# discord/lilliput

Measured on NVIDIA H100. Metric: images_per_sec_1080p_jpeg_to_256x256_jpeg_q85, higher is better.
Workload: dtype u8

## Files before the change

lilliput_b200/csrc/abi_opencv.cu:

```cuda
#include <algorithm>
#include <cstring>
#include <memory>
#include <mutex>
#include <new>
#include <string>
#include <vector>

#include "common.cuh"
#include "kernels.cuh"
#include "lp_opencv.h"

namespace lp {

thread_local long g_launches = 0;

static std::once_flag g_dev_once;
static int g_dev_status = LP_ERR_CUDA;

int ensure_device() {
    std::call_once(g_dev_once, [] {
        int n = 0;
        cudaError_t e = cudaGetDeviceCount(&n);
        if (e != cudaSuccess || n == 0) {
            fprintf(stderr,
// ... 140 lines not shown
        sets.resize(kMultiscanMaxSets);
        int rc = jpeg_parse_scans(d->data, d->len, h, scans.data(), (int)scans.size(), &nscans, sets.data(),
                                  (int)sets.size(), &nsets);
        if (rc) return rc;
        const size_t visits = jpeg_multiscan_visits(h, scans.data(), nscans);
        if (visits > kMultiscanMaxVisits) {
            fprintf(stderr, "[lilliput_b200] multi-scan JPEG: %zu block visits over %d scans exceed the serial decoder's budget\n",
                    visits, nscans);
            return LP_ERR_UNSUPPORTED;
        }
    }
    cudaStream_t st = thread_stream();
    JpegDecodeItem it;
    memset(&it, 0, sizeof(it));
    it.scan_off = 0;
    it.scan_len = (uint32_t)h.scan_length;
    it.table_set = 0;
    it.width = h.width;
    it.height = h.height;
    it.ncomp = h.ncomp;
    it.mcus_x = h.mcus_x;
    it.mcus_y = h.mcus_y;
    it.restart_interval = h.restart_interval;
    uint32_t total_blocks = 0;
    for (int c = 0; c < h.ncomp; c++) {
        it.h[c] = h.comp[c].h;
        it.v[c] = h.comp[c].v;
        it.dw[c] = (h.width * h.comp[c].h + h.maxh - 1) / h.maxh;
        it.dh[c] = (h.height * h.comp[c].v + h.maxv - 1) / h.maxv;
        total_blocks += (uint32_t)h.mcus_x * h.mcus_y * h.comp[c].h * h.comp[c].v;
        memcpy(it.qt[c], h.qt[h.comp[c].tq], sizeof(it.qt[c]));
        it.td[c] = h.comp[c].td;
        it.ta[c] = h.comp[c].ta;
    }
    uint32_t tiles = 0;
    const uint32_t blocks = jpeg_item_set_window(&it, 0, 0, h.width, h.height, false, &tiles);
    if (h.multiscan) {
        it.restart_interval = 0;
        it.table_set = 0;
        it.nscans = (uint32_t)nscans;
    }
    it.frame_channels = h.ncomp == 1 ? 1 : 3;
    JpegHuffSet hs;
    jpeg_build_huff_set(h, &hs);

    uint8_t* scratch = nullptr;
    const size_t upload_len = h.multiscan ? d->len : h.scan_length;
    const size_t scan_bytes = round_up(upload_len + 16, (size_t)256);
    const size_t sets_b = round_up(sizeof(JpegHuffSet) * (size_t)(h.multiscan ? nsets : 1), (size_t)256);
    const size_t scans_b = round_up(sizeof(JpegScanDesc) * (size_t)nscans + 16, (size_t)256);
    const size_t coef_bytes = round_up((size_t)blocks * 64 * sizeof(int16_t), (size_t)256);
    const bool parallel = h.restart_interval == 0 && !h.multiscan;
    const size_t clean_b = parallel ? round_up(huff_clean_bytes(h.scan_length), (size_t)256) : 0;
    const size_t states_b = parallel ? round_up(2 * huff_nsub(h.scan_length) * 8, (size_t)256) : 0;
    const size_t nslots_b = parallel ? round_up(2 * huff_nsub(h.scan_length) * 4, (size_t)256) : 0;
    const size_t dcdiff_b = parallel ? round_up((size_t)total_blocks * 2, (size_t)256) : 0;
    const size_t total = 1024 + sets_b + scan_bytes + coef_bytes + clean_b + states_b + nslots_b +
                         dcdiff_b + scans_b;
    LP_CUDA_OK(cudaMallocAsync(&scratch, total, st));
    JpegDecodeItem* d_item = reinterpret_cast<JpegDecodeItem*>(scratch);
    JpegHuffSet* d_hs = reinterpret_cast<JpegHuffSet*>(scratch + 1024);
    uint8_t* d_scan = scratch + 1024 + sets_b;
    int16_t* d_coef = reinterpret_cast<int16_t*>(d_scan + scan_bytes);
    uint8_t* d_clean = reinterpret_cast<uint8_t*>(d_coef) + coef_bytes;
    uint8_t* d_states = d_clean + clean_b;
    uint8_t* d_nslots = d_states + states_b;
    uint8_t* d_dcdiff = d_nslots + nslots_b;
    JpegScanDesc* d_scans = reinterpret_cast<JpegScanDesc*>(d_dcdiff + dcdiff_b);
    LP_CUDA_OK(cudaMemcpyAsync(d_item, &it, sizeof(it), cudaMemcpyHostToDevice, st));
    if (h.multiscan) {
        LP_CUDA_OK(cudaMemcpyAsync(d_hs, sets.data(), sizeof(JpegHuffSet) * nsets, cudaMemcpyHostToDevice, st));
        LP_CUDA_OK(cudaMemcpyAsync(d_scans, scans.data(), sizeof(JpegScanDesc) * nscans, cudaMemcpyHostToDevice, st));
        LP_CUDA_OK(cudaMemcpyAsync(d_scan, d->data, d->len, cudaMemcpyHostToDevice, st));
    } else {
        LP_CUDA_OK(cudaMemcpyAsync(d_hs, &hs, sizeof(hs), cudaMemcpyHostToDevice, st));
        LP_CUDA_OK(cudaMemcpyAsync(d_scan, d->data + h.scan_offset, h.scan_length, cudaMemcpyHostToDevice, st));
    }
    JpegDecodeBatch b;
    b.items = d_item;
    b.tables = d_hs;
    b.scan = d_scan;
    b.coef = d_coef;
    b.frames = m->dptr();
    b.n = 1;
    b.coef_elems_total = (size_t)blocks * 64;
    b.max_tiles_per_image = (int)tiles;
    b.use_parallel_huffman = parallel;
    b.clean = d_clean;
    b.states = d_states;
    b.nslots = reinterpret_cast<uint32_t*>(d_nslots);
    b.dcdiff = reinterpret_cast<int16_t*>(d_dcdiff);
    if (h.multiscan) {
        b.n_multiscan = 1;
        b.scans = d_scans;
    }
    int rc = jpeg_decode_launch(b, st, nullptr);
    JpegDecodeItem back;
    if (!rc) {
        LP_CUDA_OK(cudaMemcpyAsync(&back, d_item, sizeof(back), cudaMemcpyDeviceToHost, st));
        rc = sync_stream();
    }
    cudaFreeAsync(scratch, st);
    if (rc) return rc;
    return back.status == 0 ? LP_OK : LP_ERR_DECODING_FAILED;
}

static int decode_png_into(const Decoder* d, Mat* m) {
    const PngHeader& h = d->png;
// ... 666 lines not shown
```

lilliput_b200/csrc/batch.cu:

```cuda
#include <algorithm>
#include <cstring>
#include <map>
#include <string>
#include <thread>
#include <unordered_map>
#include <utility>
#include <vector>

#include "common.cuh"
#include "kernels.cuh"
#include "lilliput_host.hpp"

using namespace lp;

static constexpr int kScansPerImage = 16, kSetsPerImage = 10;

namespace lp {
size_t batch_multiscan_pool_bytes(size_t n) {
    return ((kSetsPerImage * n + kMultiscanMaxSets) * sizeof(JpegHuffSet) +
            (kScansPerImage * n + kMultiscanMaxScans) * sizeof(JpegScanDesc));
}
}

struct lp_batch {
// ... 124 lines not shown
        return nullptr;
    }
    const int slots = jpeg_huff_parallel_slots();
    b->chunk = cfg->chunk > 0 ? cfg->chunk : (slots > 0 ? 3 * slots : 512);
    b->first_chunk = slots > 0 ? std::min(slots, b->chunk) : b->chunk / 2;
    b->pipe_chunk = (cfg->chunk > 0 || slots <= 0) ? b->chunk : std::min(b->chunk, 2 * slots);
    b->chunk = std::min(b->chunk, cfg->max_images);
    b->pipe_chunk = std::max(1, std::min(b->pipe_chunk, b->chunk));
    b->max_chunks = ceil_div(cfg->max_images, b->pipe_chunk) + 3;
    const size_t mcus = (size_t)ceil_div(b->W, 8) * ceil_div(b->H, 8);
    b->max_blocks_alloc = mcus * 3 + 4 * ((size_t)ceil_div(b->W, 8) + ceil_div(b->H, 8)) + 16;
    const size_t max_blocks = b->max_blocks_alloc;
    b->frame_bytes = (size_t)b->W * b->H * 3;
    b->resized_bytes = (size_t)b->out_w * b->out_h * 3;
    const size_t N = cfg->max_images;
    auto fail = [&]() -> lp_batch* { batch_free(b); return nullptr; };
#define BALLOC(ptr, bytes)                                                                      \
    if (dev_arena) {                                                                            \
        const size_t need_ = round_up((size_t)(bytes), (size_t)256);                            \
        if (dev_used + need_ > dev_bytes) return fail();                                        \
        (ptr) = reinterpret_cast<decltype(ptr)>(dev_arena + dev_used);                          \
        dev_used += need_;                                                                      \
    } else if (cudaMalloc(&(ptr), (bytes)) != cudaSuccess) {                                    \
        fprintf(stderr, "[lilliput_b200] lp_batch_create: cudaMalloc(%zu) failed\n", (size_t)(bytes)); \
        return fail();                                                                          \
    }
#define HALLOC(ptr, bytes)                                                                      \
    if (host_arena) {                                                                           \
        const size_t need_ = round_up((size_t)(bytes), (size_t)256);                            \
        if (host_used + need_ > host_bytes) return fail();                                      \
        (ptr) = reinterpret_cast<decltype(ptr)>(host_arena + host_used);                        \
        host_used += need_;                                                                     \
    } else if (cudaMallocHost(&(ptr), (bytes)) != cudaSuccess) {                                \
        return fail();                                                                          \
    }
    if (cudaStreamCreateWithFlags(&b->st, cudaStreamNonBlocking) != cudaSuccess) return fail();
    if (cudaStreamCreateWithFlags(&b->st_h2d, cudaStreamNonBlocking) != cudaSuccess) return fail();
    if (cudaStreamCreateWithFlags(&b->st_d2h, cudaStreamNonBlocking) != cudaSuccess) return fail();
    BALLOC(b->d_scan, cfg->max_in_bytes + 16 * N + 4096);
    BALLOC(b->d_items, N * sizeof(JpegDecodeItem));
    b->max_tables = (int)N;
    if (b->multiscan) {
        b->max_tables += (int)(kSetsPerImage * N) + kMultiscanMaxSets;
        b->max_scans = kScansPerImage * N + kMultiscanMaxScans;
        BALLOC(b->d_scans, b->max_scans * sizeof(JpegScanDesc));
        BALLOC(b->d_masks, (size_t)b->chunk * max_blocks * sizeof(uint64_t));
    }
    BALLOC(b->d_tables, (size_t)b->max_tables * sizeof(JpegHuffSet));
    BALLOC(b->d_coef, (size_t)b->chunk * max_blocks * 64 * sizeof(int16_t));
    BALLOC(b->d_frames, (size_t)b->chunk * b->frame_bytes + 256);
    BALLOC(b->d_resized, N * b->resized_bytes + 256);
    BALLOC(b->d_enc_scratch, jpeg_encode_scratch_bytes(b->out_w, b->out_h, 3, b->chunk, cfg->out_cap, b->progressive));
    BALLOC(b->d_clean, cfg->max_in_bytes + 64 * N + 4096);
    b->state_cap = (cfg->max_in_bytes / 128 + 2 * N + 16) * 2;
    BALLOC(b->d_states, b->state_cap * 8);
    BALLOC(b->d_nslots, b->state_cap * 4);
    BALLOC(b->d_dcdiff, (size_t)b->chunk * max_blocks * sizeof(int16_t));
    BALLOC(b->d_out, N * cfg->out_cap);
    BALLOC(b->d_out_len, N * sizeof(uint32_t));
#undef BALLOC
    HALLOC(b->h_out, N * cfg->out_cap);
    HALLOC(b->h_out_len, N * sizeof(uint32_t));
    HALLOC(b->h_items_back, N * sizeof(JpegDecodeItem));
    HALLOC(b->h_off, (N + (size_t)b->max_chunks + 8) * sizeof(unsigned long long));
#undef HALLOC
    b->ev.resize((size_t)b->max_chunks * 6);
    b->ev_h2d.resize(b->max_chunks);
    b->ev_d2h.resize(b->max_chunks);
    for (auto& e : b->ev)
        if (cudaEventCreate(&e) != cudaSuccess) return fail();
    for (auto& e : b->ev_h2d)
        if (cudaEventCreateWithFlags(&e, cudaEventDisableTiming) != cudaSuccess) return fail();
    for (auto& e : b->ev_d2h)
        if (cudaEventCreateWithFlags(&e, cudaEventDisableTiming) != cudaSuccess) return fail();
    b->items.resize(N);
    b->parse_status.resize(N);
    b->file_dev_off.resize(N);
    return b;
}

extern "C" void lp_batch_destroy(lp_batch* b) {
    if (!b) return;
    DeviceGuard dev_guard(b->cfg.device);
    cudaDeviceSynchronize();
    batch_free(b);
}

static int table_set_lookup(lp_batch* b, const JpegHeader& h);
static int table_set_for(lp_batch* b, const JpegHeader& h) {
    if (b->last_table_idx >= 0 && !memcmp(h.huff_present, b->last_present, sizeof(h.huff_present)) &&
        !memcmp(h.huff_bits, b->last_bits, sizeof(h.huff_bits)) && !memcmp(h.huff_vals, b->last_vals, sizeof(h.huff_vals)))
        return b->last_table_idx;
    const int found = table_set_lookup(b, h);
    if (found >= 0) {
        memcpy(b->last_present, h.huff_present, sizeof(h.huff_present));
        memcpy(b->last_bits, h.huff_bits, sizeof(h.huff_bits));
        memcpy(b->last_vals, h.huff_vals, sizeof(h.huff_vals));
        b->last_table_idx = found;
    }
    return found;
}

static int table_set_lookup(lp_batch* b, const JpegHeader& h) {
    std::string key;
    for (int tc = 0; tc < 2; tc++)
        for (int th = 0; th < 4; th++) {
            key.push_back((char)h.huff_present[tc][th]);
// ... 112 lines not shown
    lay.ordinal = ordinal;
    for (int k = i0; k < i0 + cnt; k++) {
        if (b->parse_status[k]) continue;
        const JpegDecodeItem& it = b->items[k];
        lay.blocks = std::max(lay.blocks, blocks_of[k - i0]);
        lay.tiles = std::max(lay.tiles, tiles_of[k - i0]);
        lay.total_blocks = std::max(lay.total_blocks, total_of[k - i0]);
        if (!b->layout_known) {
            b->win_w = it.win_w;
            b->win_h = it.win_h;
            b->win_x0 = it.win_x0;
            b->frame_bytes = (size_t)it.win_stride * it.win_h;
            b->layout_known = true;
        }
    }
    b->blocks = std::max(b->blocks, lay.blocks);
    b->total_blocks = std::max(b->total_blocks, lay.total_blocks);
    b->chunk_layout[i0] = lay;
    for (int k = i0; k < i0 + cnt; k++) {
        if (b->parse_status[k]) continue;
        JpegDecodeItem& it = b->items[k];
        const int slot = k - i0;
        if (!ms_scans[slot].empty()) {
            const std::vector<JpegScanDesc>& sc = ms_scans[slot];
            const std::vector<JpegHeader>& sets = ms_sets[slot];
            std::vector<int> global(sets.size(), -1);
            bool fits = b->scans.size() + sc.size() <= b->max_scans;
            for (size_t q = 0; q < sets.size() && fits; q++) fits = (global[q] = table_set_for(b, sets[q])) >= 0;
            if (!fits) {
                b->parse_status[k] = LP_ERR_UNSUPPORTED;
                it.status = -1;
                continue;
            }
            it.table_set = (uint32_t)b->scans.size();
            it.nscans = (uint32_t)sc.size();
            for (JpegScanDesc d : sc) {
                d.table_set = global[d.table_set];
                b->scans.push_back(d);
            }
            it.scan_off = b->file_dev_off[k];
            it.coef_off = (uint64_t)slot * lay.blocks * 64;
            it.frame_off = (uint64_t)slot * b->frame_bytes;
            it.dcdiff_off = (uint64_t)slot * lay.total_blocks;
            b->chunk_layout[i0].n_multiscan++;
            continue;
        }
        const int ts = table_set_for(b, hdr[k - i0]);
        if (ts < 0) {
            b->parse_status[k] = LP_ERR_UNSUPPORTED;
            it.status = -1;
            continue;
        }
        it.table_set = (uint32_t)ts;
        size_t state_need = 2 * huff_nsub(it.scan_len);
        if (it.restart_interval) {
            const uint32_t mcus = (uint32_t)it.mcus_x * it.mcus_y;
            const uint32_t nint = (mcus + (uint32_t)it.restart_interval - 1) / (uint32_t)it.restart_interval;
            it.clean_len = nint;
            state_need = std::max(state_need, (size_t)nint + 2);
            if (b->state_off + state_need > b->state_cap) {
                b->parse_status[k] = LP_ERR_UNSUPPORTED;
                it.status = -1;
                continue;
            }
            for (uint32_t q = 0; q < nint; q++) b->chunk_layout[i0].rst_work.push_back(make_uint2((unsigned)slot, q));
        }
        it.scan_off = b->file_dev_off[k] + hdr[k - i0].scan_offset;
        it.coef_off = (uint64_t)slot * lay.blocks * 64;
        it.frame_off = (uint64_t)slot * b->frame_bytes;
        it.dcdiff_off = (uint64_t)slot * lay.total_blocks;
        it.clean_off = b->clean_off;
        it.state_off = b->state_off;
        b->clean_off += huff_clean_bytes(it.scan_len);
        b->state_off += state_need;
    }
    return LP_OK;
}

static int batch_upload_files(lp_batch* b, const uint8_t* const* in, const size_t* in_len, int i0, int cnt,
                              cudaStream_t st) {
    int i = i0;
    while (i < i0 + cnt) {
        int j = i;
        size_t run = in_len[i];
        while (j + 1 < i0 + cnt && in[j + 1] == in[j] + in_len[j]) { j++; run += in_len[j]; }
        LP_CUDA_OK(cudaMemcpyAsync(b->d_scan + b->file_dev_off[i], in[i], run, cudaMemcpyHostToDevice, st));
        i = j + 1;
    }
    return LP_OK;
}

static int batch_upload_items(lp_batch* b, int i0, int cnt, cudaStream_t st) {
    LP_CUDA_OK(cudaMemcpyAsync(b->d_items + i0, b->items.data() + i0, (size_t)cnt * sizeof(JpegDecodeItem),
                               cudaMemcpyHostToDevice, st));
    if (b->tables.size() > b->tables_uploaded) {
        LP_CUDA_OK(cudaMemcpyAsync(b->d_tables + b->tables_uploaded, b->tables.data() + b->tables_uploaded,
                                   (b->tables.size() - b->tables_uploaded) * sizeof(JpegHuffSet),
                                   cudaMemcpyHostToDevice, st));
        b->tables_uploaded = b->tables.size();
    }
    if (b->scans.size() > b->scans_uploaded) {
        LP_CUDA_OK(cudaMemcpyAsync(b->d_scans + b->scans_uploaded, b->scans.data() + b->scans_uploaded,
                                   (b->scans.size() - b->scans_uploaded) * sizeof(JpegScanDesc), cudaMemcpyHostToDevice,
                                   st));
        b->scans_uploaded = b->scans.size();
    }
    return LP_OK;
// ... 354 lines not shown
```

lilliput_b200/csrc/jpeg_huff_parallel.cu:

```cuda
#include <cstdlib>

#include "common.cuh"
#include "kernels.cuh"

namespace lp {

__device__ unsigned long long g_huff_phase[8];
#define LP_PHASE_MARK(k)                                             \
    do {                                                             \
        if (threadIdx.x == 0) {                                      \
            const long long now_ = clock64();                        \
            atomicAdd(&g_huff_phase[k], (unsigned long long)(now_ - s_tphase)); \
            s_tphase = now_;                                         \
        }                                                            \
    } while (0)

constexpr uint32_t kMinSubBits = 1024;
constexpr uint32_t kSubPerThread = 1;
#ifndef LP_HUFF_THREADS
#define LP_HUFF_THREADS 512
#endif
constexpr int kHuffThreads = LP_HUFF_THREADS;

__constant__ uint8_t c_zigzag_p[64] = {0,  1,  8,  16, 9,  2,  3,  10, 17, 24, 32, 25, 18, 11, 4,  5,
                                       12, 19, 26, 33, 40, 48, 41, 34, 27, 20, 13, 6,  7,  14, 21, 28,
                                       35, 42, 49, 56, 57, 50, 43, 36, 29, 22, 15, 23, 30, 37, 44, 51,
                                       58, 59, 52, 45, 38, 31, 39, 46, 53, 60, 61, 54, 47, 55, 62, 63};


template <int THREADS>
__device__ __forceinline__ uint32_t block_excl_scan(uint32_t v, uint32_t* total, uint32_t* warp_sums) {
    const int lane = threadIdx.x & 31, wid = threadIdx.x >> 5;
    uint32_t inc = v;
#pragma unroll
    for (int o = 1; o < 32; o <<= 1) {
        const uint32_t t = __shfl_up_sync(0xffffffffu, inc, o);
        if (lane >= o) inc += t;
    }
    if (lane == 31) warp_sums[wid] = inc;
    __syncthreads();
    if (wid == 0) {
        uint32_t s = lane < THREADS / 32 ? warp_sums[lane] : 0;
#pragma unroll
        for (int o = 1; o < 32; o <<= 1) {
            const uint32_t t = __shfl_up_sync(0xffffffffu, s, o);
            if (lane >= o) s += t;
        }
        if (lane < THREADS / 32) warp_sums[lane] = s;
    }
    __syncthreads();
    const uint32_t base = wid ? warp_sums[wid - 1] : 0;
    *total = warp_sums[THREADS / 32 - 1];
    __syncthreads();
    return base + inc - v;
}


__global__ void __launch_bounds__(kHuffThreads)
    jpeg_unstuff_kernel(JpegDecodeItem* items, const uint8_t* scan, uint8_t* clean) {
    __shared__ uint32_t warp_sums[kHuffThreads / 32];
    __shared__ uint32_t s_end;
    __shared__ __align__(16) uint8_t stage[kHuffThreads * 16 + 16];
    JpegDecodeItem& it = items[blockIdx.x];
    const uint8_t* src = scan + it.scan_off;
    const uint32_t len = it.scan_len;
    uint8_t* dst = clean + it.clean_off;
    const int tid = threadIdx.x, lane = tid & 31;
    if (it.restart_interval != 0 || it.nscans != 0) return;
    if (it.status != 0) {
        if (tid == 0) it.clean_len = 0;
        return;
    }
    if (tid == 0) s_end = len;
    __syncthreads();
    const uint32_t mis = (uint32_t)(reinterpret_cast<uintptr_t>(src) & 15);
// ... 75 lines not shown
        __syncthreads();
    }
    if (tid == 0) it.clean_len = carry;
    for (uint32_t k = tid; k < 32; k += kHuffThreads) dst[carry + k] = 0;
}


struct alignas(8) SubState {
    uint32_t p;
    uint32_t phase;
};

constexpr int kDcBits = 9, kAcBits = kHuffAcLookBits;

struct HuffShared {
    uint16_t dc_look[4][1 << kDcBits];
    uint16_t ac_look[4][1 << kAcBits];
    uint16_t ac_sub[4 * kHuffLongPrefixes][16];
    int32_t maxcode[8][18];
    int32_t valoffset[8][17];
    uint8_t vals[8][256];
    uint8_t zz[64];
    uint8_t blk_dc[16], blk_ac[16];
    uint8_t blk_comp[16], blk_bx[16], blk_by[16];
    uint32_t two_tables, n_first;
    uint32_t dcb_first, dcb_rest, acb_first, acb_rest;
};

struct BitWin {
    const uint32_t* w;
    uint32_t w0, w1;
    uint32_t nextw;
    uint32_t bo;
    __device__ __forceinline__ void init(const uint8_t* s, uint32_t p) {
        const uint32_t* base = reinterpret_cast<const uint32_t*>(s) + (p >> 5);
        w0 = __byte_perm(base[0], 0, 0x0123);
        w1 = __byte_perm(base[1], 0, 0x0123);
        nextw = base[2];
        w = base + 3;
        bo = p & 31;
    }
    __device__ __forceinline__ void refill() {
        if (bo >= 32) {
            w0 = w1;
            w1 = __byte_perm(nextw, 0, 0x0123);
            nextw = *w++;
            bo -= 32;
        }
    }
    __device__ __forceinline__ uint32_t peek() const { return __funnelshift_l(w1, w0, bo); }
    __device__ __forceinline__ void skip(int n) { bo += n; }
};

template <bool WRITE, bool TWO>
__device__ __forceinline__ void decode_span_t(const HuffShared& hs, const uint8_t* s, uint32_t& p, uint32_t limit,
                                            uint32_t end_bits, uint32_t& phase, uint32_t& nslots, int nb,
                                            uint64_t pos, uint64_t total_slots, const JpegDecodeItem* it,
                                            int16_t* coef, int16_t* dcdiff, int* status) {
    uint32_t blk = phase >> 6, z = phase & 63;
    const uint32_t z_start = z;
    uint32_t closed = 0;
    int32_t bits_left = (int32_t)(limit - p);
    const int32_t own_floor = (int32_t)limit - (int32_t)end_bits;
    bool own = z_start == 0;
    BitWin bw;
    bw.init(s, p);
    int16_t* dstblk = nullptr;
    bool inside = false;
    int16_t* dcp = nullptr;
    int mx = 0, my = 0;
    uint32_t blocks_left = 0;
    bool bad = false;
    int16_t* coef_base = nullptr;
    const uint32_t zzb = (uint32_t)__cvta_generic_to_shared(&hs.zz[0]);
    auto set_mcu = [&]() {
        const int rmx = mx - it->roi_mx0, rmy = my - it->roi_my0, rcx = it->roi_mcx;
        inside = (unsigned)rmx < (unsigned)rcx && (unsigned)rmy < (unsigned)it->roi_mcy;
        dstblk = coef_base + ((size_t)rmy * rcx + rmx) * ((size_t)nb * 64);
    };
    if (WRITE) {
        if (pos >= total_slots) {
            nslots = 0;
            return;
        }
        blocks_left = (uint32_t)((total_slots - pos + z_start) >> 6);
        coef_base = coef + it->coef_off;
        const uint32_t mcu = (uint32_t)((pos >> 6) / (uint32_t)nb);
        const uint32_t mcus_x = (uint32_t)it->mcus_x;
        mx = (int)(mcu % mcus_x);
        my = (int)(mcu / mcus_x);
        set_mcu();
        dstblk += blk * 64;
        dcp = dcdiff + (pos >> 6);
    }
    const uint32_t n_first = hs.n_first, dcbF = hs.dcb_first, dcbR = hs.dcb_rest, acbF = hs.acb_first, acbR = hs.acb_rest;
    uint32_t dcb, acb;
    auto set_tables = [&]() {
        if (TWO) {
            dcb = blk < n_first ? dcbF : dcbR;
            acb = blk < n_first ? acbF : acbR;
        } else {
            dcb = (uint32_t)__cvta_generic_to_shared(&hs.dc_look[hs.blk_dc[blk]][0]);
            acb = (uint32_t)__cvta_generic_to_shared(&hs.ac_look[hs.blk_ac[blk]][0]);
        }
    };
    set_tables();
    while (bits_left > 0 || (WRITE && own && z != 0 && bits_left > own_floor)) {
        bw.refill();
        const uint32_t top = bw.peek();
        const bool isdc = z == 0;
        const uint32_t idx = isdc ? (top >> (32 - kDcBits)) : (top >> (32 - kAcBits));
        int e;
        asm volatile("ld.shared.s16 %0, [%1];" : "=r"(e) : "r"((isdc ? dcb : acb) + idx * 2u));
        if (__builtin_expect(e <= 0, 0)) {
            if (e < 0) {
                e = hs.ac_sub[e & 0x7FFF][(top >> (32 - kAcBits - 4)) & 15u];
            } else {
                const int t = isdc ? hs.blk_dc[blk] : 4 + hs.blk_ac[blk];
                int len = (isdc ? kDcBits : kAcBits) + 1;
                int code = (int)(top >> (32 - len));
                while (len <= 16 && code > hs.maxcode[t][len]) {
                    len++;
                    code = (int)(top >> (32 - len));
                }
                if (len <= 16) e = (len << 8) | hs.vals[t][(code + hs.valoffset[t][len]) & 0xFF];
            }
            if (e == 0) {
                if (WRITE) {
                    *status = -3;
                    break;
                }
                bw.skip(1);
                bits_left -= 1;
                continue;
            }
        }
        const int len = e >> 8, sym = e & 0xFF;
        const uint32_t r = (uint32_t)sym >> 4, sz = (uint32_t)sym & 15;
        const bool ez = (sz == 0) && !isdc;
        const uint32_t adv = ez ? (r == 15 ? 16u : 64u) : r + 1;
        const uint32_t zt = z + adv;
        const int used = len + (ez ? 0 : (int)sz);
        if (WRITE) {
            const uint32_t t2 = top << len;
            const uint32_t raw = __funnelshift_l(t2, 0u, sz);
            const int val = (int)raw + ((int)t2 >= 0 ? (int)((0xFFFFFFFFu << sz) + 1u) : 0);
            uint32_t zi;
            asm volatile("ld.shared.u8 %0, [%1];" : "=r"(zi) : "r"(zzb + ((zt - 1u) & 63u)));
            int16_t* const where = isdc ? dcp : dstblk + zi;
            const bool inblk = zt <= 64;
            bad |= !ez && !inblk;
            if (isdc && inside) {
                uint4* const q = reinterpret_cast<uint4*>(dstblk);
#pragma unroll
                for (int k = 0; k < 8; k++) q[k] = make_uint4(0, 0, 0, 0);
            }
            if (!ez && inblk && own && (isdc || inside)) *where = (int16_t)val;
        }
        bw.skip(used);
        bits_left -= used;
        const bool fin = zt >= 64;
        z = fin ? 0u : zt;
        if (WRITE) own |= fin;
        if (!WRITE) {
            closed += fin ? 1u : 0u;
            const uint32_t nxt = blk + 1 == (uint32_t)nb ? 0u : blk + 1;
            blk = fin ? nxt : blk;
            set_tables();
        } else if (fin) {
            closed++;
            blk++;
            dstblk += 64;
            if (blk == (uint32_t)nb) {
                blk = 0;
                if (++mx == it->mcus_x) {
                    mx = 0;
                    my++;
                }
                set_mcu();
            }
            set_tables();
            if (--blocks_left == 0) break;
            dcp++;
        }
    }
    if (WRITE && bad) *status = -3;
    p = limit - (uint32_t)bits_left;
    phase = (blk << 6) | z;
    nslots = closed * 64 + z - z_start;
}

template <bool WRITE>
__device__ __forceinline__ void decode_span(const HuffShared& hs, const uint8_t* s, uint32_t& p, uint32_t limit,
                                            uint32_t end_bits, uint32_t& phase, uint32_t& nslots, int nb,
                                            uint64_t pos, uint64_t total_slots, const JpegDecodeItem* it,
                                            int16_t* coef, int16_t* dcdiff, int* status) {
    if (hs.two_tables)
        decode_span_t<WRITE, true>(hs, s, p, limit, end_bits, phase, nslots, nb, pos, total_slots, it, coef, dcdiff, status);
    else
        decode_span_t<WRITE, false>(hs, s, p, limit, end_bits, phase, nslots, nb, pos, total_slots, it, coef, dcdiff, status);
}

__device__ __forceinline__ void dc_prefix_pass(const JpegDecodeItem& it, int16_t* coef, const int16_t* dcdiff, int nb,
                                               uint32_t* warp_sums) {
    const int tid = threadIdx.x;
    constexpr int kDcRun = 8;
    const uint32_t mcus_x = (uint32_t)it.mcus_x;
    const int roi_mx0 = it.roi_mx0, roi_my0 = it.roi_my0, roi_mcx = it.roi_mcx, roi_mcy = it.roi_mcy;
    int koff = 0;
    for (int c = 0; c < it.ncomp; c++) {
        const uint32_t bpc = (uint32_t)(it.h[c] * it.v[c]);
        const uint32_t nblk = mcus_x * (uint32_t)it.mcus_y * bpc;
        const int16_t* dsrc = dcdiff + koff;
        int16_t* cdst = coef + it.coef_off + (size_t)koff * 64;
        uint32_t dc_before = 0;
        for (uint32_t base = 0; base < nblk; base += kHuffThreads * kDcRun) {
            const uint32_t j0 = base + (uint32_t)tid * kDcRun;
            const uint32_t mcu0 = j0 / bpc, kk0 = j0 % bpc;
            int d[kDcRun];
            uint32_t sum = 0;
            {
                uint32_t mcu = mcu0, kk = kk0;
#pragma unroll
                for (int r = 0; r < kDcRun; r++) {
                    d[r] = j0 + r < nblk ? dsrc[(size_t)mcu * nb + kk] : 0;
                    sum += (uint32_t)d[r];
                    if (++kk == bpc) {
                        kk = 0;
                        mcu++;
                    }
                }
            }
            uint32_t total;
            const uint32_t ex = block_excl_scan<kHuffThreads>(sum, &total, warp_sums);
            uint32_t run = dc_before + ex;
            dc_before += total;
            uint32_t mcu = mcu0, kk = kk0;
            int mx = (int)(mcu0 % mcus_x) - roi_mx0, my = (int)(mcu0 / mcus_x) - roi_my0;
#pragma unroll
            for (int r = 0; r < kDcRun; r++) {
                run += (uint32_t)d[r];
                if (j0 + r < nblk && (unsigned)mx < (unsigned)roi_mcx && (unsigned)my < (unsigned)roi_mcy)
                    cdst[(((size_t)my * roi_mcx + mx) * nb + kk) * 64] = (int16_t)(int)run;
                if (++kk == bpc) {
                    kk = 0;
                    mcu++;
                    if (++mx == (int)mcus_x - roi_mx0) {
                        mx = -roi_mx0;
                        my++;
                    }
                }
            }
        }
// ... 39 lines not shown
            bool two = true;
            for (int b = 0; b < k; b++) {
                const int ref = b < nfirst ? 0 : nfirst;
                if (hs.blk_dc[b] != hs.blk_dc[ref] || hs.blk_ac[b] != hs.blk_ac[ref]) two = false;
            }
            const int rest = nfirst < k ? nfirst : 0;
            hs.two_tables = two;
            hs.n_first = (uint32_t)nfirst;
            hs.dcb_first = (uint32_t)__cvta_generic_to_shared(&hs.dc_look[hs.blk_dc[0]][0]);
            hs.acb_first = (uint32_t)__cvta_generic_to_shared(&hs.ac_look[hs.blk_ac[0]][0]);
            hs.dcb_rest = (uint32_t)__cvta_generic_to_shared(&hs.dc_look[hs.blk_dc[rest]][0]);
            hs.acb_rest = (uint32_t)__cvta_generic_to_shared(&hs.ac_look[hs.blk_ac[rest]][0]);
            s_status = 0;
            s_carry = 0;
        }
    }
    __syncthreads();
    {
        const JpegHuffSet* g = tables + it.table_set;
        for (int i = tid; i < 4 * (1 << kAcBits); i += kHuffThreads) {
            const int t = i >> kAcBits, idx = i & ((1 << kAcBits) - 1);
            uint16_t e = g->look[4 + t][idx >> (kAcBits - 9)];
            if (!e) {
                for (int len = 10; len <= kAcBits; len++) {
                    const int code = idx >> (kAcBits - len);
                    if (code <= hs.maxcode[4 + t][len]) {
                        e = (uint16_t)((len << 8) | hs.vals[4 + t][(code + hs.valoffset[4 + t][len]) & 0xFF]);
                        break;
                    }
                }
            }
            hs.ac_look[t][idx] = e;
        }
        for (int i = tid; i < 4 * kHuffLongPrefixes * 16; i += kHuffThreads)
            (&hs.ac_sub[0][0])[i] = (&g->long_sub[0][0][0])[i];
    }
    __syncthreads();
    if (tid < 4 * kHuffLongPrefixes) {
        const uint32_t pfx = (tables + it.table_set)->long_prefix[tid / kHuffLongPrefixes][tid % kHuffLongPrefixes];
        if (pfx < (1u << kAcBits)) hs.ac_look[tid / kHuffLongPrefixes][pfx] = (uint16_t)(0x8000u | (uint32_t)tid);
    }
    __syncthreads();
    int nb = 0;
    for (int c = 0; c < it.ncomp; c++) nb += it.h[c] * it.v[c];
    const uint8_t* s = clean + it.clean_off;
    const uint32_t total_bits = it.clean_len * 8u;
    uint32_t kSubBits = (total_bits + kHuffThreads * sub_per_thread - 1) / (kHuffThreads * sub_per_thread);
    kSubBits = max(kMinSubBits, (kSubBits + 31u) & ~31u);
    const uint32_t nsub = (total_bits + kSubBits - 1) / kSubBits;
    SubState* st = states_all + it.state_off;
    uint32_t* ns = nslots_all + it.state_off;
    uint32_t* list_a = reinterpret_cast<uint32_t*>(st + nsub);
    uint32_t* list_b = list_a + nsub;
    const uint64_t total_slots = (uint64_t)it.mcus_x * it.mcus_y * nb * 64;
    int16_t* dcdiff = dcdiff_all + it.dcdiff_off;

    LP_PHASE_MARK(0);
    for (uint32_t i = tid; i < nsub; i += kHuffThreads) {
        uint32_t p = i * kSubBits, phase = 0, n = 0;
        const uint32_t limit = min((i + 1) * kSubBits, total_bits);
        decode_span<false>(hs, s, p, limit, total_bits, phase, n, nb, 0, 0, nullptr, nullptr, nullptr, nullptr);
        st[i] = SubState{p, phase};
        ns[i] = n;
    }
    __syncthreads();
    LP_PHASE_MARK(1);
    uint32_t* cur_list = list_a;
    uint32_t* nxt_list = list_b;
    uint32_t cur_count = nsub > 0 ? nsub - 1 : 0;
    bool first_round = true;
    uint32_t rounds = 0;
    while (cur_count > 0) {
        rounds++;
        if (tid == 0) s_carry = 0;
        __syncthreads();
        for (uint32_t k = tid; k < cur_count; k += kHuffThreads) {
            const uint32_t i = first_round ? k + 1 : cur_list[k];
            const uint64_t in64 = *reinterpret_cast<volatile uint64_t*>(&st[i - 1]);
            const SubState in{(uint32_t)in64, (uint32_t)(in64 >> 32)};
            const SubState old = st[i];
            uint32_t p = in.p, phase = in.phase, n = 0;
            const uint32_t limit = min((i + 1) * kSubBits, total_bits);
            if (p < limit) decode_span<false>(hs, s, p, limit, total_bits, phase, n, nb, 0, 0, nullptr, nullptr, nullptr, nullptr);
            ns[i] = n;
            if (p != old.p || phase != old.phase) {
                *reinterpret_cast<volatile uint64_t*>(&st[i]) = ((uint64_t)phase << 32) | p;
                if (i + 1 < nsub) nxt_list[atomicAdd(&s_carry, 1u)] = i + 1;
            }
        }
        __syncthreads();
        cur_count = s_carry;
        __syncthreads();
        uint32_t* t = cur_list;
        cur_list = nxt_list;
        nxt_list = t;
        first_round = false;
    }
    if (tid == 0) it.pad_ = rounds;
    LP_PHASE_MARK(2);
    SubState* cur = st;
    uint64_t slots_before = 0;
    for (uint32_t base = 0; base < nsub; base += kHuffThreads) {
        const uint32_t i = base + tid;
        const uint32_t v = i < nsub ? ns[i] : 0;
        uint32_t total;
        const uint32_t ex = block_excl_scan<kHuffThreads>(v, &total, warp_sums);
        const uint64_t pos = slots_before + ex;
        slots_before += total;
        if (i < nsub) {
            uint32_t p = i == 0 ? 0u : cur[i - 1].p;
            uint32_t phase = i == 0 ? 0u : cur[i - 1].phase;
            uint32_t n = 0;
            const uint32_t limit = min((i + 1) * kSubBits, total_bits);
            int status = 0;
            if (pos < total_slots &&
                (uint32_t)(pos % ((uint64_t)nb * 64)) != ((phase >> 6) * 64 + (phase & 63)))
                status = -3;
            if (!status && p < limit)
                decode_span<true>(hs, s, p, limit, total_bits, phase, n, nb, pos, total_slots, &it, coef, dcdiff, &status);
            if (status) s_status = status;
        }
    }
    if (tid == 0 && slots_before < total_slots) s_status = -3;
    __syncthreads();
    if (s_status) {
        if (tid == 0) it.status = s_status;
        return;
    }
    LP_PHASE_MARK(3);
    dc_prefix_pass(it, coef, dcdiff, nb, warp_sums);
    LP_PHASE_MARK(4);
    if (tid == 0) atomicAdd(&g_huff_phase[5], 1ull);
}



int jpeg_huff_phase_clocks(unsigned long long out[8], int reset) {
// ... 33 lines not shown
```

lilliput_b200/csrc/kernels.cuh:

```cuda
#pragma once
#include <cuda_runtime.h>

#include <cstddef>
#include <cstdint>
#include <vector>

#include "jpeg_types.h"

namespace lp {

struct ResizeArgs {
    const uint8_t* src;
    size_t src_img_stride, src_row_stride;
    int channels;
    int crop_x, crop_y, crop_w, crop_h;
    uint8_t* dst;
    size_t dst_img_stride, dst_row_stride;
    int dst_w, dst_h;
    int n;
    int interpolation;
};
int resize_launch(const ResizeArgs& a, cudaStream_t st);

struct JpegComp {
// ... 5 lines not shown
    int maxh = 1, maxv = 1;
    uint16_t qt[4][64];
    bool qt_present[4] = {false, false, false, false};
    uint8_t huff_bits[2][4][17];
    uint8_t huff_vals[2][4][256];
    bool huff_present[2][4] = {{false, false, false, false}, {false, false, false, false}};
    int restart_interval = 0;
    int orientation = 1;
    size_t scan_offset = 0;
    size_t scan_length = 0;
    bool progressive = false;
    bool supported = false;
    bool multiscan = false;
    int mcus_x = 0, mcus_y = 0;
};
int jpeg_parse_header(const uint8_t* data, size_t len, JpegHeader* out);



uint32_t jpeg_item_set_window(JpegDecodeItem* it, int x0, int y0, int x1, int y1, bool align16,
                              uint32_t* tiles);

void jpeg_build_huff_set(const JpegHeader& h, JpegHuffSet* out);
int jpeg_parse_scans(const uint8_t* data, size_t len, const JpegHeader& h, JpegScanDesc* scans, int max_scans,
                     int* nscans, JpegHeader* sets, int max_sets, int* nsets);
int jpeg_parse_scans(const uint8_t* data, size_t len, const JpegHeader& h, JpegScanDesc* scans, int max_scans,
                     int* nscans, JpegHuffSet* sets, int max_sets, int* nsets);
constexpr int kMultiscanMaxScans = 256, kMultiscanMaxSets = 64;
constexpr size_t kMultiscanMaxVisits = (size_t)1 << 26;
size_t jpeg_multiscan_visits(const JpegHeader& h, const JpegScanDesc* scans, int nscans);

struct JpegDecodeBatch {
    JpegDecodeItem* items;
    const JpegHuffSet* tables;
    const uint8_t* scan;
    int16_t* coef;
    uint8_t* frames;
    int n;
    size_t coef_elems_total;
    int max_tiles_per_image;
    bool use_parallel_huffman = false;
    uint8_t* clean = nullptr;
    void* states = nullptr;
    uint32_t* nslots = nullptr;
    int16_t* dcdiff = nullptr;
    int n_multiscan = 0;
    const JpegScanDesc* scans = nullptr;
    uint64_t* masks = nullptr;
    const uint2* rst_work = nullptr;
    int n_rst_work = 0;
};
inline size_t huff_clean_bytes(size_t scan_len) { return ((scan_len + 48 + 15) / 16) * 16; }
inline size_t huff_nsub(size_t scan_len) { return scan_len * 8 / 1024 + 2; }
struct JpegHuffParallelArgs {
    JpegDecodeItem* items;
    const JpegHuffSet* tables;
    const uint8_t* scan;
    uint8_t* clean;
    void* states;
    uint32_t* nslots;
    int16_t* coef;
    int16_t* dcdiff;
    int n;
};
int jpeg_huff_parallel_launch(const JpegHuffParallelArgs& a, cudaStream_t st);
int jpeg_huff_parallel_slots();
int jpeg_huff_phase_clocks(unsigned long long out[8], int reset);
int jpeg_decode_launch(const JpegDecodeBatch& b, cudaStream_t st, cudaEvent_t ev_after_huff);

struct PngSegment {
    size_t offset, length;
};
struct PngHeader {
    int width = 0, height = 0, bit_depth = 0, color_type = 0, interlace = 0;
    int src_channels = 0, out_channels = 0, bpp = 1;
    size_t row_bytes = 0;
    int npal = 0, ntrns = 0;
    bool has_trns = false;
    uint8_t palette[256 * 3] = {0};
    uint8_t trns[256] = {0};
    uint16_t trns_rgb[3] = {0, 0, 0};
    std::vector<PngSegment> idat;
    size_t idat_total = 0;
    int orientation = 1;
};
bool exif_orientation_opencv(const uint8_t* tiff, size_t n, int* value);
int png_parse(const uint8_t* data, size_t len, PngHeader* out);
int png_extract_icc(const uint8_t* data, size_t len, uint8_t* dest, size_t dest_len);
int png_extract_cicp(const uint8_t* data, size_t len, uint8_t* out4);

struct PngDecodeItem {
    uint64_t z_off, raw_off, frame_off;
    uint32_t z_len;
    int32_t width, height, bit_depth, color_type, src_channels, out_channels, bpp;
    uint32_t row_bytes, frame_stride;
    int32_t npal, ntrns, has_trns;
    uint16_t trns_rgb[3];
    uint16_t pad_;
    uint8_t palette[256 * 3];
    uint8_t trns[256];
    int32_t status;
    uint32_t produced;
    int32_t interlace, npass;
    uint32_t raw_total;
    uint32_t pass_off[7], pass_rb[7];
    int32_t pass_w[7], pass_h[7];
// ... 83 lines not shown
```

lilliput_b200/csrc/xbatch.cu:

```cuda
#include <algorithm>
#include <atomic>
#include <chrono>
#include <condition_variable>
#include <cstring>
#include <map>
#include <memory>
#include <mutex>
#include <thread>
#include <tuple>
#include <vector>

#include "common.cuh"
#include "kernels.cuh"
#include "lilliput_host.hpp"
#include "lp_opencv.h"

using namespace lp;

namespace lp {
lp_batch* batch_create_in(const lp_batch_config* cfg, uint8_t* dev_arena, size_t dev_bytes, uint8_t* host_arena,
                          size_t host_bytes, bool progressive_jpeg, bool multiscan_sources);
size_t batch_multiscan_pool_bytes(size_t n);
}

// ... 660 lines not shown
        for (int i : idx) push_fallback(X, i);
        return;
    }
    std::vector<uint8_t> file;
    for (int a = 0; a < na; a++) {
        const int i = idx[a];
        bool good = st[a] == 0;
        for (int f = first[a]; f < first[a + 1] && good; f++) good = !frames[f].image.empty();
        if (!good) {
            push_fallback(X, i);
            continue;
        }
        uint32_t bg = 0xFFFFFFFFu;
        int loops = 0;
        gif_plan_info(X->items[i].gif, nullptr, nullptr, nullptr, &bg, &loops);
        for (int f = first[a]; f < first[a + 1]; f++) {
            frames[f].duration = gif_plan_delay_ms(X->items[i].gif, f - first[a]);
            L.d2h += frames[f].image.size() + frames[f].alph.size();
        }
        webp_assemble(&frames[first[a]], first[a + 1] - first[a], nullptr, 0, bg, (uint32_t)loops, &file);
        if (file.size() > X->out_cap) {
            X->status[i] = LP_ERR_INVALID_IMAGE;
            X->out_len[i] = 0;
            continue;
        }
        memcpy(X->out[i], file.data(), file.size());
        X->out_len[i] = file.size();
        X->status[i] = LP_OK;
    }
}


static void run_jpeg(lp_xbatch* X, Lane& L, const std::vector<int>& idx) {
    const int n = (int)idx.size();
    const XItem& g = X->items[idx[0]];
    size_t in_bytes = 0;
    for (int i : idx) in_bytes += X->in_len[i];
    lp_batch_config c;
    memset(&c, 0, sizeof(c));
    c.device = X->device;
    c.max_images = n;
    c.src_width = g.w;
    c.src_height = g.h;
    c.dst_width = X->opt.width;
    c.dst_height = X->opt.height;
    c.resize_method = X->opt.resize_method;
    c.jpeg_quality = X->quality;
    c.max_in_bytes = in_bytes + (1 << 20);
    c.out_cap = std::min(X->out_cap, round_up(std::max((size_t)65536, (size_t)g.ow * g.oh * 3), (size_t)256));
    if (c.out_cap >= 256) c.out_cap = c.out_cap / 256 * 256;
    const size_t mcus = (size_t)ceil_div(g.w, 8) * ceil_div(g.h, 8);
    const size_t per_img = (mcus * 3 + 64) * (128 + 64 + 2 + (g.jpeg_multiscan ? 8 : 0)) + (size_t)g.w * g.h * 3 + 65536;
    const size_t pools = g.jpeg_multiscan ? batch_multiscan_pool_bytes((size_t)n) : 0;
    const size_t fixed = 2 * in_bytes + (size_t)n * (c.out_cap + (size_t)g.ow * g.oh * 3 + 4096) + (64u << 20) + pools;
    const int slots = jpeg_huff_parallel_slots();
    long fit = L.dev_bytes > fixed ? (long)((L.dev_bytes - fixed) / per_img) : 0;
    if (fit < 1) {
        for (int i : idx) push_fallback(X, i);
        return;
    }
    int chunk = (int)std::min<long>(fit, 3L * std::max(slots, 1));
    if (slots > 0 && chunk > slots) chunk = chunk / slots * slots;
    c.chunk = std::max(1, std::min(chunk, n));
    lp_batch* b = batch_create_in(&c, L.dev, L.dev_bytes, L.host, L.host_bytes, X->progressive, g.jpeg_multiscan);
    if (!b) {
        for (int i : idx) push_fallback(X, i);
        return;
    }
    std::vector<const uint8_t*> in((size_t)n);
    std::vector<size_t> len((size_t)n), olen((size_t)n, 0);
    std::vector<uint8_t*> out((size_t)n);
    std::vector<int> st((size_t)n, 0);
    for (int k = 0; k < n; k++) {
        in[k] = X->in[idx[k]];
        len[k] = X->in_len[idx[k]];
        out[k] = X->out[idx[k]];
    }
    cudaEventRecord(L.ev[0], L.st);
    const int rc = lp_batch_transform(b, in.data(), len.data(), n, out.data(), olen.data(), st.data());
    L.h2d += in_bytes;
    for (int k = 0; k < n; k++) {
        const int i = idx[k];
        if (rc || st[k] != LP_OK) {
            push_fallback(X, i);
            continue;
        }
        X->out_len[i] = olen[k];
        X->status[i] = LP_OK;
        L.d2h += olen[k];
    }
    lp_batch_destroy(b);
}


extern "C" lp_xbatch* lp_xbatch_create(const lp_xbatch_config* cfg) {
    if (!cfg) return nullptr;
    if (ensure_device()) return nullptr;
    int prev = 0;
    cudaGetDevice(&prev);
    if (cudaSetDevice(cfg->device) != cudaSuccess) return nullptr;
    lp_xbatch* X = new lp_xbatch;
    X->cfg = *cfg;
    X->device = cfg->device;
    memset(&X->stats, 0, sizeof(X->stats));
    unsigned hc = std::thread::hardware_concurrency();
    X->threads = cfg->host_threads > 0 ? cfg->host_threads : (int)std::min(16u, std::max(2u, hc));
    size_t free_b = 0, total_b = 0;
// ... 351 lines not shown
```

Baseline: 51350.

## Add checkpoint rejoin to parallel Huffman sync passes to stop re-decoding converged spans

During the parallel Huffman synchronisation rounds, each subsequence now records decoder state checkpoints every fixed number of bits on the first pass. In later passes a re-decode compares its state against the stored checkpoint and stops early once it matches, adjusting the slot counts incrementally. The goal is to cut redundant re-decoding work in the self-synchronisation loop. It costs extra state memory, sized through new helpers in both the single-image and batch allocations, plus per-symbol checkpoint checks in the hot loop.

Result: faster. 52260, median of 6 (+1.8%).

```diff
diff --git a/lilliput_b200/csrc/abi_opencv.cu b/lilliput_b200/csrc/abi_opencv.cu
--- a/lilliput_b200/csrc/abi_opencv.cu
+++ b/lilliput_b200/csrc/abi_opencv.cu
@@ -216,8 +216,8 @@
     const size_t coef_bytes = round_up((size_t)blocks * 64 * sizeof(int16_t), (size_t)256);
     const bool parallel = h.restart_interval == 0 && !h.multiscan;
     const size_t clean_b = parallel ? round_up(huff_clean_bytes(h.scan_length), (size_t)256) : 0;
-    const size_t states_b = parallel ? round_up(2 * huff_nsub(h.scan_length) * 8, (size_t)256) : 0;
-    const size_t nslots_b = parallel ? round_up(2 * huff_nsub(h.scan_length) * 4, (size_t)256) : 0;
+    const size_t states_b = parallel ? round_up(huff_state_entries(h.scan_length) * 8, (size_t)256) : 0;
+    const size_t nslots_b = parallel ? round_up(huff_state_entries(h.scan_length) * 4, (size_t)256) : 0;
     const size_t dcdiff_b = parallel ? round_up((size_t)total_blocks * 2, (size_t)256) : 0;
     const size_t total = 1024 + sets_b + scan_bytes + coef_bytes + clean_b + states_b + nslots_b +
                          dcdiff_b + scans_b;
diff --git a/lilliput_b200/csrc/batch.cu b/lilliput_b200/csrc/batch.cu
--- a/lilliput_b200/csrc/batch.cu
+++ b/lilliput_b200/csrc/batch.cu
@@ -200,7 +200,7 @@
     BALLOC(b->d_resized, N * b->resized_bytes + 256);
     BALLOC(b->d_enc_scratch, jpeg_encode_scratch_bytes(b->out_w, b->out_h, 3, b->chunk, cfg->out_cap, b->progressive));
     BALLOC(b->d_clean, cfg->max_in_bytes + 64 * N + 4096);
-    b->state_cap = (cfg->max_in_bytes / 128 + 2 * N + 16) * 2;
+    b->state_cap = huff_batch_state_entries(cfg->max_in_bytes, N);
     BALLOC(b->d_states, b->state_cap * 8);
     BALLOC(b->d_nslots, b->state_cap * 4);
     BALLOC(b->d_dcdiff, (size_t)b->chunk * max_blocks * sizeof(int16_t));
@@ -419,7 +419,7 @@
             continue;
         }
         it.table_set = (uint32_t)ts;
-        size_t state_need = 2 * huff_nsub(it.scan_len);
+        size_t state_need = huff_state_entries(it.scan_len);
         if (it.restart_interval) {
             const uint32_t mcus = (uint32_t)it.mcus_x * it.mcus_y;
             const uint32_t nint = (mcus + (uint32_t)it.restart_interval - 1) / (uint32_t)it.restart_interval;
diff --git a/lilliput_b200/csrc/jpeg_huff_parallel.cu b/lilliput_b200/csrc/jpeg_huff_parallel.cu
--- a/lilliput_b200/csrc/jpeg_huff_parallel.cu
+++ b/lilliput_b200/csrc/jpeg_huff_parallel.cu
@@ -21,6 +21,7 @@
 #define LP_HUFF_THREADS 512
 #endif
 constexpr int kHuffThreads = LP_HUFF_THREADS;
+
 
 __constant__ uint8_t c_zigzag_p[64] = {0,  1,  8,  16, 9,  2,  3,  10, 17, 24, 32, 25, 18, 11, 4,  5,
                                        12, 19, 26, 33, 40, 48, 41, 34, 27, 20, 13, 6,  7,  14, 21, 28,
@@ -202,14 +203,24 @@
     __device__ __forceinline__ void skip(int n) { bo += n; }
 };
 
-template <bool WRITE, bool TWO>
+constexpr int kCkRecord = 1, kCkRejoin = 2;
+struct Checkpoints {
+    SubState* cp;
+    uint32_t* cn;
+    uint32_t next;
+    uint32_t replaced;
+    bool rejoined;
+};
+
+template <bool WRITE, bool TWO, int CK>
 __device__ __forceinline__ void decode_span_t(const HuffShared& hs, const uint8_t* s, uint32_t& p, uint32_t limit,
                                             uint32_t end_bits, uint32_t& phase, uint32_t& nslots, int nb,
                                             uint64_t pos, uint64_t total_slots, const JpegDecodeItem* it,
-                                            int16_t* coef, int16_t* dcdiff, int* status) {
+                                            int16_t* coef, int16_t* dcdiff, int* status, Checkpoints* ck) {
     uint32_t blk = phase >> 6, z = phase & 63;
     const uint32_t z_start = z;
     uint32_t closed = 0;
+    uint32_t ck_next = CK ? ck->next : 0, ck_slots = 0;
     int32_t bits_left = (int32_t)(limit - p);
     const int32_t own_floor = (int32_t)limit - (int32_t)end_bits;
     bool own = z_start == 0;
@@ -256,6 +267,25 @@
     };
     set_tables();
     while (bits_left > 0 || (WRITE && own && z != 0 && bits_left > own_floor)) {
+        if (CK) {
+            const uint32_t at = limit - (uint32_t)bits_left;
+            if (at >= ck_next) {
+                const uint32_t j = ck_next / kHuffCheckBits - 1, ph = (blk << 6) | z, slots = closed * 64 + z - z_start;
+                if (CK == kCkRejoin) {
+                    const SubState old = ck->cp[j];
+                    ck->replaced += ck->cn[j];
+                    if (old.p == at && old.phase == ph) {
+                        ck->cn[j] = slots - ck_slots;
+                        ck->rejoined = true;
+                        break;
+                    }
+                }
+                ck->cp[j] = SubState{at, ph};
+                ck->cn[j] = slots - ck_slots;
+                ck_slots = slots;
+                ck_next += kHuffCheckBits;
+            }
+        }
         bw.refill();
         const uint32_t top = bw.peek();
         const bool isdc = z == 0;
@@ -335,20 +365,29 @@
         }
     }
     if (WRITE && bad) *status = -3;
+    if (CK && !ck->rejoined) {
+        const uint32_t slots = closed * 64 + z - z_start;
+        for (; ck_next < limit; ck_next += kHuffCheckBits) {
+            const uint32_t j = ck_next / kHuffCheckBits - 1;
+            ck->cp[j] = SubState{limit - (uint32_t)bits_left, (blk << 6) | z};
+            ck->cn[j] = slots - ck_slots;
+            ck_slots = slots;
+        }
+    }
     p = limit - (uint32_t)bits_left;
     phase = (blk << 6) | z;
     nslots = closed * 64 + z - z_start;
 }
 
-template <bool WRITE>
+template <bool WRITE, int CK = 0>
 __device__ __forceinline__ void decode_span(const HuffShared& hs, const uint8_t* s, uint32_t& p, uint32_t limit,
                                             uint32_t end_bits, uint32_t& phase, uint32_t& nslots, int nb,
                                             uint64_t pos, uint64_t total_slots, const JpegDecodeItem* it,
-                                            int16_t* coef, int16_t* dcdiff, int* status) {
+                                            int16_t* coef, int16_t* dcdiff, int* status, Checkpoints* ck = nullptr) {
     if (hs.two_tables)
-        decode_span_t<WRITE, true>(hs, s, p, limit, end_bits, phase, nslots, nb, pos, total_slots, it, coef, dcdiff, status);
+        decode_span_t<WRITE, true, CK>(hs, s, p, limit, end_bits, phase, nslots, nb, pos, total_slots, it, coef, dcdiff, status, ck);
     else
-        decode_span_t<WRITE, false>(hs, s, p, limit, end_bits, phase, nslots, nb, pos, total_slots, it, coef, dcdiff, status);
+        decode_span_t<WRITE, false, CK>(hs, s, p, limit, end_bits, phase, nslots, nb, pos, total_slots, it, coef, dcdiff, status, ck);
 }
 
 __device__ __forceinline__ void dc_prefix_pass(const JpegDecodeItem& it, int16_t* coef, const int16_t* dcdiff, int nb,
@@ -494,6 +533,8 @@
     uint32_t* ns = nslots_all + it.state_off;
     uint32_t* list_a = reinterpret_cast<uint32_t*>(st + nsub);
     uint32_t* list_b = list_a + nsub;
+    SubState* cp = st + 2 * nsub;
+    uint32_t* cn = ns + 2 * nsub;
     const uint64_t total_slots = (uint64_t)it.mcus_x * it.mcus_y * nb * 64;
     int16_t* dcdiff = dcdiff_all + it.dcdiff_off;
 
@@ -520,11 +561,20 @@
             const uint32_t i = first_round ? k + 1 : cur_list[k];
             const uint64_t in64 = *reinterpret_cast<volatile uint64_t*>(&st[i - 1]);
             const SubState in{(uint32_t)in64, (uint32_t)(in64 >> 32)};
+            uint32_t p = in.p, phase = in.phase, n = 0;
+            Checkpoints ck{cp, cn, i * kSubBits + kHuffCheckBits, 0, false};
+            if (first_round)
+                decode_span<false, kCkRecord>(hs, s, p, min((i + 1) * kSubBits, total_bits), total_bits, phase, n, nb, 0, 0,
+                                              nullptr, nullptr, nullptr, nullptr, &ck);
+            else
+                decode_span<false, kCkRejoin>(hs, s, p, min((i + 1) * kSubBits, total_bits), total_bits, phase, n, nb, 0, 0,
+                                          nullptr, nullptr, nullptr, nullptr, &ck);
+            if (ck.rejoined) {
+                ns[i] += n - ck.replaced;
+                continue;
+            }
+            ns[i] = n;
             const SubState old = st[i];
-            uint32_t p = in.p, phase = in.phase, n = 0;
-            const uint32_t limit = min((i + 1) * kSubBits, total_bits);
-            if (p < limit) decode_span<false>(hs, s, p, limit, total_bits, phase, n, nb, 0, 0, nullptr, nullptr, nullptr, nullptr);
-            ns[i] = n;
             if (p != old.p || phase != old.phase) {
                 *reinterpret_cast<volatile uint64_t*>(&st[i]) = ((uint64_t)phase << 32) | p;
                 if (i + 1 < nsub) nxt_list[atomicAdd(&s_carry, 1u)] = i + 1;
diff --git a/lilliput_b200/csrc/kernels.cuh b/lilliput_b200/csrc/kernels.cuh
--- a/lilliput_b200/csrc/kernels.cuh
+++ b/lilliput_b200/csrc/kernels.cuh
@@ -81,6 +81,10 @@
 };
 inline size_t huff_clean_bytes(size_t scan_len) { return ((scan_len + 48 + 15) / 16) * 16; }
 inline size_t huff_nsub(size_t scan_len) { return scan_len * 8 / 1024 + 2; }
+constexpr uint32_t kHuffCheckBits = 2048;
+static_assert(kHuffCheckBits % 32 == 0 && kHuffCheckBits >= 512, "checkpoints sit on word boundaries, many symbols apart");
+inline size_t huff_state_entries(size_t scan_len) { return 2 * huff_nsub(scan_len) + scan_len * 8 / kHuffCheckBits; }
+inline size_t huff_batch_state_entries(size_t in_bytes, size_t n) { return huff_state_entries(in_bytes) + huff_state_entries(0) * n + 32; }
 struct JpegHuffParallelArgs {
     JpegDecodeItem* items;
     const JpegHuffSet* tables;
diff --git a/lilliput_b200/csrc/xbatch.cu b/lilliput_b200/csrc/xbatch.cu
--- a/lilliput_b200/csrc/xbatch.cu
+++ b/lilliput_b200/csrc/xbatch.cu
@@ -736,7 +736,9 @@
     const size_t mcus = (size_t)ceil_div(g.w, 8) * ceil_div(g.h, 8);
     const size_t per_img = (mcus * 3 + 64) * (128 + 64 + 2 + (g.jpeg_multiscan ? 8 : 0)) + (size_t)g.w * g.h * 3 + 65536;
     const size_t pools = g.jpeg_multiscan ? batch_multiscan_pool_bytes((size_t)n) : 0;
-    const size_t fixed = 2 * in_bytes + (size_t)n * (c.out_cap + (size_t)g.ow * g.oh * 3 + 4096) + (64u << 20) + pools;
+    const size_t states = (8 + 4) * huff_batch_state_entries(c.max_in_bytes, (size_t)n);
+    const size_t fixed = 2 * in_bytes + (size_t)n * (c.out_cap + (size_t)g.ow * g.oh * 3 + 4096) + (64u << 20) + pools +
+                         states;
     const int slots = jpeg_huff_parallel_slots();
     long fit = L.dev_bytes > fixed ? (long)((L.dev_bytes - fixed) / per_img) : 0;
     if (fit < 1) {
```
